# manixq/stereo_matchin

Hardware: AMD Instinct MI355X
Metric: disparity maps/sec + ms/frame, 1920×1080 d=256 ASW win=35, 1/2/4/8 MI355X (higher is better)
Workload: dtype f32

## Files before the change

include/asw.h:

```cpp
#ifndef ASW_H
#define ASW_H

#include <stddef.h>
#include <stdint.h>

#ifdef __cplusplus
extern "C" {
#endif

#define ASW_OK 0
#define ASW_E_INVALID -1
#define ASW_E_HIP -2
#define ASW_E_NOMEM -3
#define ASW_E_UNSUPPORTED -4
#define ASW_E_COMM -5

#define ASW_DIR_V 0
#define ASW_DIR_H 1

#define ASW_COLOR_RGB 0
#define ASW_COLOR_LAB 1

#define ASW_LR_U8 0
#define ASW_LR_NATIVE 1
// ... 153 lines not shown
void asw_refine_params_default(asw_refine_params *rp);
int asw_refine_params_check(const asw_params *p, const asw_refine_params *rp);
size_t asw_refine_lut_bytes(const asw_refine_params *rp);
int asw_refine_lut(const asw_params *p, const asw_refine_params *rp, float *lut, void *stream);

int asw_ref_v(const asw_params *p, const asw_refine_params *rp, const uint8_t *img_rgba, const uint8_t *est,
              int est_stride, const float *conf, const float *lut, float *out, void *stream);
int asw_ref_h(const asw_params *p, const asw_refine_params *rp, const uint8_t *img_rgba, const float *conf,
              const float *in, const float *lut, float *out, void *stream);
int asw_wta_ref(const asw_params *p, const float *cost, const float *ref_l, const float *ref_r, int32_t *d_ref,
                int32_t *d_tar, float *conf_ref, uint8_t *code_ref, uint8_t *code_tar, void *stream);
int asw_median3(const asw_params *p, const uint8_t *codes, int stride, uint8_t *out_rgba, void *stream);

size_t asw_refine_workspace_bytes(const asw_params *p, const asw_refine_params *rp);
int asw_refine(const asw_params *p, const asw_refine_params *rp, const uint8_t *left_rgba, const uint8_t *right_rgba,
               const float *cost, uint8_t *est_left_rgba, uint8_t *code_tar, float *conf_ref, float *conf_tar,
               void *workspace, uint8_t *post_red_rgba, uint8_t *final_rgba, int32_t *d_ref, int32_t *d_tar,
               void *stream);

int asw_refine_native_params_check(const asw_params *p, const asw_refine_params *rp);
int asw_refine_native_lut(const asw_params *p, const asw_refine_params *rp, float *lut, void *stream);
int asw_ref_v_native(const asw_params *p, const asw_refine_params *rp, const uint8_t *img_rgba, const int32_t *est,
                     const float *conf, const float *lut, float *out, void *stream);
int asw_consistency_native(const asw_params *p, const int32_t *d_ref, const int32_t *d_tar, float *conf_ref,
                           float *conf_tar, int32_t *est_left, uint16_t *post16, void *stream);
int asw_median3_u16(const asw_params *p, const int32_t *in, uint16_t *out, void *stream);
size_t asw_refine_native_workspace_bytes(const asw_params *p, const asw_refine_params *rp);
int asw_refine_native(const asw_params *p, const asw_refine_params *rp, const uint8_t *left_rgba,
                      const uint8_t *right_rgba, const float *cost, int32_t *est_left, int32_t *d_tar, float *conf_ref,
                      float *conf_tar, void *workspace, uint16_t *post16, uint16_t *final16, int32_t *d_ref,
                      void *stream);

typedef struct asw_cross_params {
    int arm_max;
    int tau;
} asw_cross_params;
void asw_cross_params_default(asw_cross_params *cp);
int asw_cross_params_check(const asw_params *p, const asw_cross_params *cp);
size_t asw_cross_arm_bytes(const asw_params *p);
int asw_median3_rgba(const asw_params *p, const uint8_t *in_rgba, uint8_t *out_rgba, void *stream);
int asw_cross_arms(const asw_params *p, const asw_cross_params *cp, const uint8_t *med_rgba, int8_t *arms,
                   void *stream);
int asw_cross_cost(const asw_params *p, const uint8_t *med_left_rgba, const uint8_t *med_right_rgba, float *cost,
                   void *stream);
int asw_cross_integral(const asw_params *p, int dir, float *vol, void *stream);
int asw_cross_oii(const asw_params *p, int dir, const int8_t *arms_left, const int8_t *arms_right, const float *in,
                  float *out, void *stream);
int asw_cross_init(const asw_params *p, const float *vol, int32_t *d0, uint8_t *code0, void *stream);
int asw_cross_vote(const asw_params *p, const uint8_t *code0, const int8_t *arms_left, int32_t *d1, uint8_t *code1,
                   void *stream);

#define ASW_TUNE_PASS_VARIANT 1
#define ASW_TUNE_WTA_VARIANT 2
int asw_tune_set(int key, int value);
int asw_pass_kernel(int dir, int den_mode, char *buf, int len);


typedef struct asw_ctx asw_ctx;

typedef struct asw_outputs {
    int32_t *d_ref, *d_tar;
    float *conf_ref, *conf_tar;
    uint8_t *disp_rgba;
    uint8_t *lr_rgba;
    uint8_t *lr_red_rgba;
    float *cost;
    uint8_t *final_rgba;
    uint8_t *post_red_rgba;
    uint16_t *disp16;
    uint16_t *lr16;
} asw_outputs;
#define ASW_DISP16_INVALID 0xFFFF

typedef struct asw_timings {
    double raw_cost, support, v_pass_mean, h_pass_mean, aggregation_total, wta, consistency, total;
    double h2d, d2h;
    double refine;
    double exchange;
} asw_timings;

int asw_device_name(int hip_device, char *buf, int len);

int asw_create(const asw_params *p, int hip_device, asw_ctx **out);
int asw_create_multi(const asw_params *p, const int *hip_device_ids, int n_devices, asw_ctx **out);
#define ASW_COMM_ID_BYTES 128
int asw_comm_unique_id(uint8_t id[ASW_COMM_ID_BYTES]);
int asw_create_rank(const asw_params *p, int hip_device, int rank, int nranks, const uint8_t id[ASW_COMM_ID_BYTES],
                    asw_ctx **out);
int asw_ctx_shard(const asw_ctx *ctx, int i, int *n_shards, int *d_begin, int *d_end);
int asw_destroy(asw_ctx *ctx);
int asw_match(asw_ctx *ctx, const uint8_t *left_rgba, const uint8_t *right_rgba, asw_outputs *out,
              asw_timings *t);
int asw_match_batch(asw_ctx *ctx, const uint8_t *left_rgba, const uint8_t *right_rgba, int batch,
                    asw_outputs *out, asw_timings *t);
int asw_set_refine(asw_ctx *ctx, const asw_refine_params *rp);
typedef struct asw_refine_native_outputs {
    uint16_t *final16;
    uint16_t *post16;
    int32_t *d_ref, *d_tar;
} asw_refine_native_outputs;
int asw_set_refine_native(asw_ctx *ctx, const asw_refine_params *rp, const asw_refine_native_outputs *o);
int asw_set_graph(asw_ctx *ctx, int on);
typedef struct asw_subpixel_outputs {
    float *disp;
    float *disp_lr;
    float *disp_filled;
// ... 31 lines not shown
```

stereo_matchin_amd/csrc/asw_aggregate.hip:

```cpp
#include <hip/hip_runtime.h>

#include <cstdio>
#include <cstring>
#include <mutex>

#include "asw_common.h"

namespace asw {
namespace agg {
int g_pass_variant = 0;
template <int T, int DM>
int launch_pass_tm(const asw_params *p, int dir, const float *wl, const float *wr, const float *cin, float *cout,
                   float *den, hipStream_t st, const RawSrc *raw);
template <int T, int DM>
int launch_pass32_tm(const asw_params *p, int dir, const float *wl, const float *wr, const float *cin, float *cout,
                     float *den, hipStream_t st);
template <int T, int DM>
int launch_pass32_c16_tm(const asw_params *p, const float *wl, const float *wr, const uint16_t *cin16, float *cout,
                         float *den, hipStream_t st);
template <int T>
int launch_pass32_t(const asw_params *p, int dir, const float *wl, const float *wr, const float *cin, float *cout,
                    float *den, int dm, hipStream_t st) {
    if (dm == 1) return launch_pass32_tm<T, 1>(p, dir, wl, wr, cin, cout, den, st);
    if (dm == 2) return launch_pass32_tm<T, 2>(p, dir, wl, wr, cin, cout, den, st);
    return launch_pass32_tm<T, 0>(p, dir, wl, wr, cin, cout, den, st);
}
template <int T>
int launch_pass_t(const asw_params *p, int dir, const float *wl, const float *wr, const float *cin, float *cout,
                  float *den, int dm, hipStream_t st, const RawSrc *raw) {
    if (asw_disp_pitch(p) == 32) {
        if (raw && dir == ASW_DIR_V) {
            if (dm == 1) return launch_pass32_c16_tm<T, 1>(p, wl, wr, raw->cost16, cout, den, st);
            if (dm == 0) return launch_pass32_c16_tm<T, 0>(p, wl, wr, raw->cost16, cout, den, st);
            return ASW_E_INVALID;
        }
        return launch_pass32_t<T>(p, dir, wl, wr, cin, cout, den, dm, st);
    }
    if (dm == 1) return launch_pass_tm<T, 1>(p, dir, wl, wr, cin, cout, den, st, raw);
    if (dm == 2) return launch_pass_tm<T, 2>(p, dir, wl, wr, cin, cout, den, st, raw);
    return launch_pass_tm<T, 0>(p, dir, wl, wr, cin, cout, den, st, raw);
}
}

int launch_pass_any(const asw_params *p, int dir, const float *wl, const float *wr, const float *cin, float *cout,
                    float *den, int dm, hipStream_t st);

int set_pass_variant(int v) {
    const int old = agg::g_pass_variant;
    agg::g_pass_variant = v;
    return old;
}

namespace {
std::mutex g_note_mu;
char g_note[2][3][96];
}

void note_pass_kernel(int dir, int dm, const char *kernel, int T, const char *shape, bool nt) {
    if (dir < 0 || dir > 1 || dm < 0 || dm > 2) return;
    std::lock_guard<std::mutex> lk(g_note_mu);
    std::snprintf(g_note[dir][dm], sizeof g_note[dir][dm], "%s<T=%d,%s,DM=%d%s>", kernel, T, shape, dm,
                  nt ? ",nt" : "");
}

int pass_shape_check(const asw_params *p) {
    const long long rowbytes = (long long)p->width * asw_disp_pitch(p) * 4;
    if (rowbytes * (2LL * p->taps + 16) >= (1LL << 31)) return ASW_E_UNSUPPORTED;
    if ((long long)asw_support_bytes(p) >= (1LL << 31)) return ASW_E_UNSUPPORTED;
    return ASW_OK;
}

bool ring_taps(int T) {
#ifdef ASW_DEV_TAPS
    return T == ASW_DEV_TAPS;
#else
    return T == 3 || T == 5 || T == 7 || T == 9 || T == 15 || T == 33 || T == 35 || T == 51;
#endif
}

int launch_pass(const asw_params *p, int dir, const float *wl, const float *wr, const float *cin, float *cout,
                float *den, int dm, hipStream_t st, const RawSrc *raw) {
    if (dm != 0 && !den) return ASW_E_INVALID;
    if (const int s = pass_shape_check(p)) return s;
    if (raw && (dir != ASW_DIR_V || dm == 2 || !ring_taps(p->taps))) return ASW_E_UNSUPPORTED;
#ifdef ASW_DEV_TAPS
    if (p->taps == ASW_DEV_TAPS) return agg::launch_pass_t<ASW_DEV_TAPS>(p, dir, wl, wr, cin, cout, den, dm, st, raw);
    if (raw) return ASW_E_UNSUPPORTED;
    return launch_pass_any(p, dir, wl, wr, cin, cout, den, dm, st);
#endif
    switch (p->taps) {
#define ASW_CASE(TT) \
    case TT:         \
        return agg::launch_pass_t<TT>(p, dir, wl, wr, cin, cout, den, dm, st, raw);
        ASW_CASE(3)
        ASW_CASE(5)
        ASW_CASE(7)
        ASW_CASE(9)
        ASW_CASE(15)
        ASW_CASE(33)
        ASW_CASE(35)
        ASW_CASE(51)
#undef ASW_CASE
// ... 29 lines not shown
```

stereo_matchin_amd/csrc/asw_aggregate_impl.h:

```cpp
#pragma once
#include <hip/hip_runtime.h>

#include <cstdint>
#include <type_traits>

#include "asw_common.h"

namespace asw {
namespace agg {

using f4 = float __attribute__((ext_vector_type(4)));

__device__ __forceinline__ int clampi(int v, int lo, int hi) { return v < lo ? lo : (v > hi ? hi : v); }

constexpr int kPS = 4;
constexpr int kPW = 4;

template <int B, int E, class F>
__device__ __forceinline__ void static_for(F &&f) {
    if constexpr (B < E) {
        f(std::integral_constant<int, B>{});
        static_for<B + 1, E>(f);
    }
}

__device__ __forceinline__ float div_pos(float num, float den) {
    float r = __builtin_amdgcn_rcpf(den);
    const float e = __builtin_fmaf(-den, r, 1.0f);
    r = __builtin_fmaf(e, r, r);
    float q = num * r;
    float rem = __builtin_fmaf(-den, q, num);
    q = __builtin_fmaf(rem, r, q);
    rem = __builtin_fmaf(-den, q, num);
    return __builtin_fmaf(rem, r, q);
}

template <int T>
struct Halves {
    static constexpr int QT = (T + 3) / 4;
    static constexpr int QA = (QT + 1) / 2;
    static constexpr int TA = 4 * QA < T ? 4 * QA : T;
    static constexpr int TB = T - TA;
    static constexpr int QB = QT - QA;
    static constexpr int NA = TA, NB = TB > 0 ? TB : 1;
    static constexpr int MA = QA, MB = QB > 0 ? QB : 1;
};

template <int T, int NPH>
struct Phases {
    static constexpr int QT = (T + 3) / 4;
    static constexpr int gb(int k) { return (QT * k + NPH - 1) / NPH; }
    static constexpr int tb(int k) { return 4 * gb(k) < T ? 4 * gb(k) : T; }
    static constexpr int NG = (QT + NPH - 1) / NPH;
    static constexpr int NT = 4 * NG;
};

template <int N>
__device__ __forceinline__ void wait_lgkm() {
    static_assert(N >= 0 && N < 16, "lgkmcnt field");
// ... 145 lines not shown
        const float *wlx = wlrow + xb * TP + s * TP;
        const f4 *wrx = my_slab + (xb - xs) * Q + s * Q;
        wait_lgkm0();
        asm volatile("" ::"v"(win[(s + T - 1) % U]));
        __builtin_amdgcn_sched_barrier(0);
        if constexpr (HV::TB > 0) {
            load_wl<HV::TA, T>(wlb, wlx);
            read_wr<T, HV::QA, HV::QT>(wrb, wrx);
        }
        __builtin_amdgcn_sched_barrier(0);
        float num = 1e-5f, dn = 1e-5f;
        taps<U, s, 0, HV::TA, DM != DM_READ>(num, dn, wla, wra, win);
        __builtin_amdgcn_sched_barrier(0);
        wait_lgkm0();
        __builtin_amdgcn_sched_barrier(0);
        {
            const float *pn;
            if constexpr (CHK || s == U - 1) pn = wlrow + min(x + 1, W - 1) * TP;
            else pn = wlx + TP;
            load_wl<0, HV::TA>(wla, pn);
            read_wr<T, 0, HV::QA>(wra, wrx + Q);
        }
        __builtin_amdgcn_sched_barrier(0);
        if constexpr (HV::TB > 0) taps<U, s, HV::TA, T, DM != DM_READ>(num, dn, wlb, wrb, win);
        const int xo = x * xstride;
        if constexpr (DM == DM_READ) {
            dn = dring[s % 2];
            dring[s % 2] = bload<CP>(rd, voff, min(x + 2, W - 1) * xstride);
        } else if constexpr (DM == DM_WRITE) {
            bstore<CP>(dn, rd, voff, xo);
        }
        bstore<CP>(div_pos(num, dn), ro, voff, xo);
        win[(s + U - 1) % U] = bload<CP>(rc, voff, min(x + R + P, W - 1) * xstride);
        sink += warm[s % PW];
        warm[s % PW] = wlrow[min(x + 1 + PW, W - 1) * TP + warm_off];
    };
    int xb = xw0;
    for (; xb + U <= xw1; xb += U)
        static_for<0, U>([&](auto sc) __attribute__((always_inline)) { body(sc, std::false_type{}, xb); });
    if (xb < xw1)
        static_for<0, U>([&](auto sc) __attribute__((always_inline)) { body(sc, std::true_type{}, xb); });
    if (sink == -1.0f) cout[rowoff] = sink;
}


constexpr int h11_batch(int T, int NKW) {
    return pf9_period(T) % 8 == 0 && 8 * (tap_pitch(T) / 4) <= 64 * NKW ? 8 : 4;
}
constexpr int h11_ring(int T, int NKW) { return (64 * NKW + 2 * h11_batch(T, NKW) + 15) / 16 * 16; }

template <int T, int NKW, int DM, int CP, int CPS = CP, int PX = 0, int KDH = 4>
__global__ __launch_bounds__(64 * NKW) __attribute__((amdgpu_waves_per_eu(T > 35 ? 3 : 4))) void k_hpass11(
    const float *__restrict__ wl, const float *__restrict__ wr, const float *__restrict__ cin,
    float *__restrict__ cout, float *__restrict__ den, int W, int H, int Dp, int d_begin, int nseg, int seg_len,
    int groups_per_xcd, int ngroups, int ring_off, int kbg0, int nkbg) {
    constexpr int R = T / 2;
    constexpr int TP = tap_pitch(T);
    constexpr int Q = TP / 4;
    constexpr int U = pf9_period(T) + PX;
    constexpr int P = U - T;
    constexpr int PW = 4;
    constexpr int KD = KDH;
    static_assert(U % KD == 0, "den ring period");
    constexpr int NT = 64 * NKW;
    constexpr int K = h11_batch(T, NKW);
    constexpr int RING = h11_ring(T, NKW);
    constexpr int EB = Q * 16;
    constexpr int RB = RING * EB;
    static_assert(U % K == 0 && RING >= NT + 2 * K && RING % 16 == 0, "ring geometry");
    static_assert(K * Q <= NT, "one staged float4 per thread per batch");
    __shared__ f4 ring[RING * Q];

    const int xcd = blockIdx.x & 7, m = blockIdx.x >> 3;
    const int gl = m / nkbg;
    const int g = xcd * groups_per_xcd + gl;
    if (gl >= groups_per_xcd || g >= ngroups) return;
    const int kbg = kbg0 + m - gl * nkbg;
    const int y = g / nseg;
    const int xs = (g - y * nseg) * seg_len;
    const int xe = min(xs + seg_len, W);
    const int lane = threadIdx.x & 63;
    const int wave = __builtin_amdgcn_readfirstlane(threadIdx.x >> 6);
    const int d0 = d_begin + kbg * NT;
    const int kb = kbg * NT + wave * 64;
    const float *wrrow = wr + (long long)y * W * TP;

    {
        const int e0 = xs - d0 - (NT - 1);
        for (int t = threadIdx.x; t < (NT + K) * Q; t += NT) {
            const int e = t / Q, q = t - e * Q;
            const int xr = e0 + e;
            ring[((xr + ring_off) % RING) * Q + q] =
                *reinterpret_cast<const f4 *>(wrrow + clampi(xr, 0, W - 1) * TP + 4 * q);
        }
    }
    const int st_t = min((int)threadIdx.x, K * Q - 1);
    const int st_e = st_t / Q, st_q = st_t - st_e * Q;
    int st_xr = xs + K + 1 - d0 + st_e;
    int st_addr = ((st_xr + ring_off) % RING) * EB + st_q * 16;
    f4 stg = *reinterpret_cast<const f4 *>(wrrow + clampi(st_xr, 0, W - 1) * TP + 4 * st_q);
    __syncthreads();

    const long long rowoff = (long long)y * W * Dp + kb;
    const rsrc_t rc = make_rsrc(cin + rowoff);
    const rsrc_t ro = make_rsrc(cout + rowoff);
    const rsrc_t rd = make_rsrc(den + rowoff);
    const int voff = lane * 4;
    const int xstride = Dp * 4;
    const float *wlrow = wl + (long long)y * W * TP;
    const int warm_off = lane < TP ? lane : 0;
    int ra = ((xs - d0 - wave * 64 - lane + ring_off) % RING) * EB;
    auto ring_next = [](int a) __attribute__((always_inline)) {
        const unsigned t = (unsigned)a + EB, u = t - (unsigned)RB;
        return (int)(t < u ? t : u);
    };
    auto at = [&](int a) __attribute__((always_inline)) {
        return reinterpret_cast<const f4 *>(reinterpret_cast<const char *>(ring) + a);
    };

    using HV = Halves<T>;
    float win[U];
    float wla[HV::NA], wlb[HV::NB];
    f4 wra[HV::MA], wrb[HV::MB];
    float warm[PW];
    float dring[KD];
    float sink = 0.0f;
#pragma unroll
    for (int j = 0; j < U - 1; ++j) win[j] = bload<CP>(rc, voff, clampi(xs - R + j, 0, W - 1) * xstride);
    if constexpr (DM == DM_READ) {
#pragma unroll
        for (int j = 0; j < KD; ++j) dring[j] = bload<CP>(rd, voff, min(xs + j, W - 1) * xstride);
    }
#pragma unroll
    for (int j = 0; j < PW; ++j) warm[j] = wlrow[min(xs + 1 + j, W - 1) * TP + warm_off];
    load_wl<0, HV::TA>(wla, wlrow + xs * TP);
    read_wr<T, 0, HV::QA>(wra, at(ra));

    auto body = [&](auto sc, auto chk, int xb) __attribute__((always_inline)) {
        constexpr int s = decltype(sc)::value;
        constexpr bool CHK = decltype(chk)::value;
        const int x = xb + s;
        if constexpr (CHK) {
            if (x >= xe) return;
        }
        const float *wlx = wlrow + xb * TP + s * TP;
        if constexpr (s % K == 0) {
            __syncthreads();
            *reinterpret_cast<f4 *>(reinterpret_cast<char *>(ring) + st_addr) = stg;
            st_xr += K;
            st_addr += K * EB;
            st_addr = st_addr >= RB ? st_addr - RB : st_addr;
            stg = *reinterpret_cast<const f4 *>(wrrow + clampi(st_xr, 0, W - 1) * TP + 4 * st_q);
        } else {
            wait_lgkm0();
        }
        asm volatile("" ::"v"(win[(s + T - 1) % U]));
        __builtin_amdgcn_sched_barrier(0);
        if constexpr (HV::TB > 0) {
            load_wl<HV::TA, T>(wlb, wlx);
            read_wr<T, HV::QA, HV::QT>(wrb, at(ra));
        }
        __builtin_amdgcn_sched_barrier(0);
        float num = 1e-5f, dn = 1e-5f;
        taps<U, s, 0, HV::TA, DM != DM_READ>(num, dn, wla, wra, win);
        __builtin_amdgcn_sched_barrier(0);
        wait_lgkm0();
        __builtin_amdgcn_sched_barrier(0);
        ra = ring_next(ra);
        {
            const float *pn;
            if constexpr (CHK || s == U - 1) pn = wlrow + min(x + 1, W - 1) * TP;
            else pn = wlx + TP;
            load_wl<0, HV::TA>(wla, pn);
            read_wr<T, 0, HV::QA>(wra, at(ra));
        }
        __builtin_amdgcn_sched_barrier(0);
        if constexpr (HV::TB > 0) taps<U, s, HV::TA, T, DM != DM_READ>(num, dn, wlb, wrb, win);
        const int xo = x * xstride;
        if constexpr (DM == DM_READ) {
            dn = dring[s % KD];
            dring[s % KD] = bload<CP>(rd, voff, min(x + KD, W - 1) * xstride);
        } else if constexpr (DM == DM_WRITE) {
            bstore<CPS>(dn, rd, voff, xo);
        }
        bstore<CPS>(div_pos(num, dn), ro, voff, xo);
        win[(s + U - 1) % U] = bload<CP>(rc, voff, min(x + R + P, W - 1) * xstride);
        sink += warm[s % PW];
        warm[s % PW] = wlrow[min(x + 1 + PW, W - 1) * TP + warm_off];
    };
    int xb = xs;
    for (; xb + U <= xe; xb += U)
        static_for<0, U>([&](auto sc) __attribute__((always_inline)) { body(sc, std::false_type{}, xb); });
    if (xb < xe)
        static_for<0, U>([&](auto sc) __attribute__((always_inline)) { body(sc, std::true_type{}, xb); });
    if (sink == -1.0f) cout[rowoff] = sink;
}



constexpr int ring_div(int U, int lo) {
    int n = lo;
    while (U % n != 0) ++n;
    return n;
}
constexpr int cmax(int a, int b) { return a > b ? a : b; }

template <int T, int NW, int DM, int RB, int CP, int CPS = CP, int KDV = 2, int PSV = 4, int TK = 0, int NPH = 2,
          int PX = 0, int WPE = 0, bool C16 = false>
__global__ __launch_bounds__(NW * 64) __attribute__((amdgpu_waves_per_eu(WPE ? WPE : NW >= 16 ? 4 : NW >= 12 ? 3 : 2))) void k_vpass10(
    const float *__restrict__ wl, const float *__restrict__ wr, const float *__restrict__ cin, float *__restrict__ cout,
    float *__restrict__ den, int W, int H, int Dp, int d_begin, int rows_per_strip, int nxb, int nstrip,
    int xg_per_xcd) {
    constexpr int R = T / 2;
    constexpr int TP = tap_pitch(T);
    constexpr int Q = TP / 4;
    constexpr int U = pf9_period(T) + PX;
    constexpr int P = U - T;
    constexpr int PS = PSV;
    constexpr int PW = 4;
    constexpr int KD = KDV;
    constexpr int LEAD = RB + 1;
    constexpr int NBUF = ring_div(U, 2 * RB + 1);
    static_assert(U % PS == 0 && U % PW == 0 && U % KD == 0 && U % RB == 0 && U % NBUF == 0, "ring periods");
    static_assert(LEAD <= PS, "staging ring too short for the barrier period");
    constexpr int LA = cmax(cmax(R + P, LEAD + PS), cmax(PW, KD));
    constexpr int SLAB = NW + 63;
    constexpr int NQ = SLAB * Q;
    constexpr int NSTAGE = (NQ + NW * 64 - 1) / (NW * 64);
    static_assert(NSTAGE <= 2, "slab row larger than two float4 per thread");
    __shared__ f4 slab[NBUF][NQ];

    const int nkb = Dp / 64;
    const int xcd = blockIdx.x & 7, m = blockIdx.x >> 3;
    int xg, kbi, strip;
    if constexpr (TK > 0) {
        constexpr int TCG = 32 / TK;
        const int j = m % 32, t = m / 32;
        const int ntk = (nkb + TK - 1) / TK, ntc = (xg_per_xcd + TCG - 1) / TCG;
        const int tk = t % ntk, rest = t / ntk;
        const int cgl = (rest % ntc) * TCG + j % TCG;
        kbi = tk * TK + j / TCG;
        strip = rest / ntc;
        if (cgl >= xg_per_xcd || kbi >= nkb) return;
        xg = xcd * xg_per_xcd + cgl;
    } else {
        xg = xcd * xg_per_xcd + m % xg_per_xcd;
        const int rest = m / xg_per_xcd;
// ... 155 lines not shown
                if constexpr (k == 0 && s % RB == 0) __syncthreads();
                else wait_lgkm0();
                if constexpr (k == 0) asm volatile("" ::"v"(win[(s + T - 1) % U]));
                __builtin_amdgcn_sched_barrier(0);
                if constexpr (k + 1 < NPH) {
                    request(std::integral_constant<int, k + 1>{}, wo, bcur);
                } else {
                    if constexpr (CLAMP) {
                        wo = min(y + 1, H - 1) * wrow;
                    } else {
                        wo += wrow;
                        asm volatile("" : "+s"(wo));
                    }
                    request(std::integral_constant<int, 0>{}, wo, bnext);
                }
                if constexpr (k == 0) {
                    put(bput, sa[(s + LEAD) % PS], sb[(s + LEAD) % PS]);
                    stage(sa[(s + LEAD) % PS], sb[(s + LEAD) % PS],
                          CLAMP ? min(y + LEAD + PS, H - 1) * wrow_b : soff);
                }
                __builtin_amdgcn_sched_barrier(0);
                taps<U, s, PH::tb(k), PH::tb(k + 1), DM != DM_READ>(num, dn, wlp[k], wrp[k], win);
                __builtin_amdgcn_sched_barrier(0);
            });
            if constexpr (DM == DM_READ) {
                dn = dring[s % KD];
                dring[s % KD] = bload<CP>(rdn, voff,
                                          CLAMP ? (min(y + KD, H - 1) - min(ys + KD, H - 1)) * rowbytes : so);
            } else if constexpr (DM == DM_WRITE) {
                bstore<CPS>(dn, rd, voff, so);
            }
            bstore<CPS>(div_pos(num, dn), ro, voff, so);
            if constexpr (C16) r16[s % PR] = cload_raw(rc, CLAMP ? (min(y + R + P, H - 1) - cb) * rowbytes : so);
            else win[(s + U - 1) % U] = cload(rc, CLAMP ? (min(y + R + P, H - 1) - cb) * rowbytes : so);
            sink += warm[s % PW];
            warm[s % PW] = bload(rwl, warm_voff, CLAMP ? min(y + PW, H - 1) * wrow_b : woff);
            so += rowbytes;
            woff += wrow_b;
            soff += wrow_b;
            asm volatile("" : "+s"(so), "+s"(woff), "+s"(soff));
        });
    };
    int ys = y_begin;
    for (; ys + U <= y_end && ys + U - 1 + LA <= H - 1; ys += U) chunk(std::integral_constant<int, 0>{}, ys);
    for (; ys + U <= y_end; ys += U) {
        asm volatile("" : "+s"(ys));
        chunk(std::integral_constant<int, 1>{}, ys);
    }
    if (ys < y_end) chunk(std::integral_constant<int, 2>{}, ys);
    if (sink == -1.0f) cout[kb + lane] = sink;
}

extern int g_pass_variant;

template <int T, int NW, int DM, int RB = 2, int CP = 0, int CPS = CP, int PS = 4, int NPH = 2, bool C16 = false,
          int TK = 0>
void launch_v10(const asw_params *p, const float *wl, const float *wr, const float *cin, float *cout, float *den,
                hipStream_t st, const RawSrc *raw = nullptr) {
    constexpr int U = pf9_period(T);
    const int W = p->width, H = p->height;
    const int Dp = asw_disp_pitch(p);
    const int nkb = Dp / 64;
    const int nxb = (W + NW - 1) / NW;
    int nstrip = (int)((2048LL + (long long)nxb * nkb - 1) / ((long long)nxb * nkb));
    const int max_strip = H / (2 * T) > 1 ? H / (2 * T) : 1;
    if (nstrip > max_strip) nstrip = max_strip;
    if (nstrip < 1) nstrip = 1;
    const int rows = ((H + nstrip - 1) / nstrip + U - 1) / U * U;
    nstrip = (H + rows - 1) / rows;
    const int per_xcd = (nxb + 7) / 8;
    constexpr int TCG = TK > 0 ? 32 / TK : 1;
    const int nblocks = TK > 0 ? 8 * 32 * ((nkb + TK - 1) / (TK > 0 ? TK : 1)) * ((per_xcd + TCG - 1) / TCG) * nstrip
                               : 8 * per_xcd * nkb * nstrip;
    hipLaunchKernelGGL((k_vpass10<T, NW, DM, RB, CP, CPS, 2, PS, TK, NPH, 0, 0, C16>), dim3(nblocks), dim3(NW * 64), 0,
                       st, wl, wr, C16 ? reinterpret_cast<const float *>(raw->cost16) : cin, cout, den, W, H, Dp,
                       p->d_begin, rows, nxb, nstrip, per_xcd);
    const char *shape = NW == 16 ? (NPH == 2 ? "NW=16" : "NW=16,NPH>2")
                        : NW == 12 ? (NPH == 2 ? "NW=12" : TK == 4 ? "NW=12,NPH=3,TK=4" : "NW=12,NPH=3") : "NW=8";
    note_pass_kernel(ASW_DIR_V, DM, C16 ? "k_vpass10_c16" : "k_vpass10", T, shape, CP == kCPStream);
}

template <int T, int NW, int XW, int DM, int CP = 0>
void launch_h9(const asw_params *p, const float *wl, const float *wr, const float *cin, float *cout, float *den,
               hipStream_t st) {
    const int W = p->width, H = p->height;
    const int Dp = asw_disp_pitch(p);
    const int nkb = Dp / 64;
    constexpr int SEG = NW * XW;
    const int nseg = (W + SEG - 1) / SEG;
    const int nblocks = (H * nseg + 7) / 8 * 8 * nkb;
    hipLaunchKernelGGL((k_hpass9<T, NW, XW, DM, CP>), dim3(nblocks), dim3(NW * 64), 0, st, wl, wr, cin, cout, den, W, H,
                       Dp, p->d_begin, nseg);
    note_pass_kernel(ASW_DIR_H, DM, "k_hpass9", T, "NW=4", CP == kCPStream);
}

template <int T, int NKW, int DM, int CP, int CPS = CP, int PX = 0, int KDH = 4>
void launch_h11(const asw_params *p, const float *wl, const float *wr, const float *cin, float *cout, float *den,
                hipStream_t st, int seg_len) {
#ifndef ASW_PASS_EXP_FORMS
    static_assert(NKW == 4 || NKW == 2 || NKW == 1, "no label for this block shape");
    static_assert(PX == 0 || (NKW == 2 && PX == 24), "the PX=24 label names the 2-block form with PX = 24");
#endif
    constexpr int RING = h11_ring(T, NKW);
    const int W = p->width, H = p->height;
    const int Dp = asw_disp_pitch(p);
    const int nkbg = Dp / (64 * NKW);
    const int nseg = (W + seg_len - 1) / seg_len;
    const int ngroups = H * nseg;
    const int per_xcd = (ngroups + 7) / 8;
    const int ring_off = ((p->d_begin + Dp) / RING + 1) * RING;
    hipLaunchKernelGGL((k_hpass11<T, NKW, DM, CP, CPS, PX, KDH>), dim3(8 * per_xcd * nkbg), dim3(64 * NKW), 0, st, wl, wr, cin,
                       cout, den, W, H, Dp, p->d_begin, nseg, seg_len, per_xcd, ngroups, ring_off, 0, nkbg);
    note_pass_kernel(ASW_DIR_H, DM, "k_hpass11", T,
                     NKW == 4 ? "NKW=4" : NKW == 2 ? (PX ? "NKW=2,PX=24" : "NKW=2") : "NKW=1", CP == kCPStream);
}

inline bool v12_tiles(const asw_params *p) {
    const int nxb = (p->width + 11) / 12;
    return asw_disp_pitch(p) / 64 >= 4 && (nxb + 7) / 8 >= 8;
}

template <int T, int DM>
void launch_dm(const asw_params *p, int dir, const float *wl, const float *wr, const float *cin, float *cout,
               float *den, hipStream_t st, const RawSrc *raw) {
    constexpr int U9 = pf9_period(T);
    constexpr int XW9 = U9 * (64 / U9 > 1 ? 64 / U9 : 1);
    const int v = g_pass_variant;
    bool stream = (long long)p->width * p->height * asw_disp_pitch(p) * 4 >= (256LL << 20);
    if (v & (1 << 26)) stream = !stream;
    if (raw) {
        if constexpr (DM != DM_READ) {
            if constexpr (T <= 35) {
                if (stream) launch_v10<T, 16, DM, 2, kCPStream, kCPStream, 4, 2, true>(p, wl, wr, cin, cout, den, st, raw);
                else launch_v10<T, 16, DM, 2, 0, 0, 4, 2, true>(p, wl, wr, cin, cout, den, st, raw);
            } else {
                if (stream && v12_tiles(p)) launch_v10<T, 12, DM, 2, kCPStream, kCPStream, 4, 3, true, 4>(p, wl, wr, cin, cout, den, st, raw);
                else if (stream) launch_v10<T, 12, DM, 2, kCPStream, kCPStream, 4, 3, true>(p, wl, wr, cin, cout, den, st, raw);
                else launch_v10<T, 12, DM, 2, 0, 0, 4, 3, true>(p, wl, wr, cin, cout, den, st, raw);
            }
        }
        return;
    }
    if (dir == ASW_DIR_V) {
        if (stream) {
            if constexpr (T <= 35) launch_v10<T, 16, DM, 2, kCPStream>(p, wl, wr, cin, cout, den, st);
            else if (v12_tiles(p)) launch_v10<T, 12, DM, 2, kCPStream, kCPStream, 4, 3, false, 4>(p, wl, wr, cin, cout, den, st);
            else launch_v10<T, 12, DM, 2, kCPStream, kCPStream, 4, 3>(p, wl, wr, cin, cout, den, st);
        } else {
            if constexpr (T <= 35) launch_v10<T, 16, DM, 2, 0>(p, wl, wr, cin, cout, den, st);
            else launch_v10<T, 12, DM, 2, 0, 0, 4, 3>(p, wl, wr, cin, cout, den, st);
        }
    } else {
        const int nkb = asw_disp_pitch(p) / 64;
        const int seg = h11_seg_len(T, v);
        if (h11_selected(p, v)) {
            if constexpr (T <= 35) {
                if (nkb % 4 == 0) launch_h11<T, 4, DM, kCPStream>(p, wl, wr, cin, cout, den, st, seg);
                else if (nkb % 2 == 0) launch_h11<T, 2, DM, kCPStream>(p, wl, wr, cin, cout, den, st, seg);
                else launch_h11<T, 1, DM, kCPStream>(p, wl, wr, cin, cout, den, st, seg);
            } else if constexpr (T == 51 && DM == DM_READ) {
                constexpr int PXH = 24;
                const int seg51 = (v >> 8) & 15 ? seg : 4 * (pf9_period(T) + PXH);
                if (nkb % 2 == 0) launch_h11<T, 2, DM, kCPStream, kCPStream, PXH>(p, wl, wr, cin, cout, den, st, seg51);
                else launch_h11<T, 1, DM, kCPStream>(p, wl, wr, cin, cout, den, st, seg);
            } else {
                if (nkb % 2 == 0) launch_h11<T, 2, DM, kCPStream>(p, wl, wr, cin, cout, den, st, seg);
                else launch_h11<T, 1, DM, kCPStream>(p, wl, wr, cin, cout, den, st, seg);
            }
        } else if (stream) {
            launch_h9<T, 4, XW9, DM, kCPStream>(p, wl, wr, cin, cout, den, st);
        } else {
            launch_h9<T, 4, XW9, DM>(p, wl, wr, cin, cout, den, st);
        }
    }
}

template <int T, int DM>
int launch_pass_tm(const asw_params *p, int dir, const float *wl, const float *wr, const float *cin, float *cout,
                   float *den, hipStream_t st, const RawSrc *raw) {
    launch_dm<T, DM>(p, dir, wl, wr, cin, cout, den, st, raw);
    const hipError_t e = hipGetLastError();
    if (e != hipSuccess) {
        set_hip_error(e);
        return ASW_E_HIP;
    }
    return ASW_OK;
}

}
}

#define ASW_INSTANTIATE_PASS(TT, DM)                                                                                 \
    template int asw::agg::launch_pass_tm<TT, DM>(const asw_params *, int, const float *, const float *,            \
                                                  const float *, float *, float *, hipStream_t, const RawSrc *);
```

stereo_matchin_amd/csrc/asw_common.h:

```cpp
#pragma once
#include <hip/hip_runtime.h>

#include "asw.h"

namespace asw {

constexpr int kWave = 64;
constexpr int kSadMax = 765;
constexpr int kLutWidth = kSadMax + 1;

__host__ __device__ constexpr int tap_pitch(int T) {
    int k = (T + 3) / 4;
    if ((k & 1) == 0) ++k;
    return 4 * k;
}

__host__ __device__ constexpr int round_up(int v, int m) { return (v + m - 1) / m * m; }

__host__ __device__ inline int code_u8(int d, int D) {
    if (D <= 1) return 0;
    long long c = (510LL * d + (D - 2)) / (2LL * (D - 1));
    return c > 255 ? 255 : (c < 0 ? 0 : (int)c);
}

__device__ __forceinline__ bool lr_consistent(int mode, int D, long long p, int dr, const int32_t *d_tar,
                                              const uint8_t *code_ref, const uint8_t *code_tar) {
    if (mode == ASW_LR_U8) {
        const float scale = (float)(D - 1);
        const float qr = ((float)code_ref[p] / 255.0f) * scale;
        const float qt = ((float)code_tar[p] / 255.0f) * scale;
        return fabsf(qt - qr) < 1.001f;
    }
    const int dd = dr - d_tar[p];
    return dd <= 1 && dd >= -1;
}

void set_hip_error(hipError_t e);

__host__ __device__ inline int d_end_of_p(const asw_params *p) { return p->d_end < 0 ? p->ndisp : p->d_end; }

struct RawSrc {
    const uint16_t *cost16;
};

int launch_pass(const asw_params *p, int dir, const float *wl, const float *wr, const float *cin, float *cout,
                float *den, int dm, hipStream_t st, const RawSrc *raw = nullptr);
int h11_seg_len(int T, int variant);
bool h11_selected(const asw_params *p, int variant);
bool ring_taps(int T);
int set_pass_variant(int v);
constexpr int kPassVariantBits = 128 | 4096 | 0xF00;
void note_pass_kernel(int dir, int dm, const char *kernel, int T, const char *shape, bool nt);
int pass_shape_check(const asw_params *p);

int raw_cost16_check(const asw_params *p);
int census_cost16_check(const asw_params *p, const asw_census_params *cp);
int sgm_shape_check(const asw_params *p);

int launch_wta_local_scan(const asw_params *p, const float *cost, const float *ref, long long *key, float *m1,
                          float *m2, hipStream_t st);
int launch_wta_target_local_scan(const asw_params *p, const float *cost, const long long *key_ref, const float *ref,
                                 long long *tkey, float *t1, float *t2, hipStream_t st);
int launch_wta_scan(const asw_params *p, int mode, const float *cost, const float *ref_l, const float *ref_r,
                    int32_t *d_ref, float *conf_ref, int32_t *d_tar, float *conf_tar, uint8_t *code_ref,
                    uint8_t *code_tar, hipStream_t st);

}
```

stereo_matchin_amd/csrc/asw_kernels.hip:

```cpp
#include <hip/hip_runtime.h>

#include <climits>
#include <cstdint>

#include "asw_common.h"
#include "asw_srgb_table.h"

namespace asw {

static thread_local int g_last_hip_error = 0;
void set_hip_error(hipError_t e) { g_last_hip_error = (int)e; }

namespace {

__device__ __forceinline__ int clampi(int v, int lo, int hi) { return v < lo ? lo : (v > hi ? hi : v); }

__device__ double exp_d(double x) {
    const double inv_ln2 = 1.44269504088896338700e+00;
    const double ln2_hi = 6.93147180369123816490e-01;
    const double ln2_lo = 1.90821492927058770002e-10;
    const double k = rint(x * inv_ln2);
    double r = fma(-k, ln2_hi, x);
    r = fma(-k, ln2_lo, r);
    double p = 1.0 / 87178291200.0;
// ... 316 lines not shown
                              uchar4 *__restrict__ out_red) {
    const long long p = (long long)blockIdx.x * blockDim.x + threadIdx.x;
    if (p >= n) return;
    const uint8_t cr = code_ref[p], ct = code_tar[p];
    bool cons;
    if (mode == ASW_LR_U8) {
        const float scale = (float)(D - 1);
        const float qr = ((float)cr / 255.0f) * scale;
        const float qt = ((float)ct / 255.0f) * scale;
        cons = fabsf(qt - qr) < 1.001f;
    } else {
        const int dd = d_ref[p] - d_tar[p];
        cons = dd <= 1 && dd >= -1;
    }
    if (!cons) {
        conf_ref[p] = 0.0f;
        conf_tar[p] = 0.0f;
    }
    if (out) out[p] = cons ? make_uchar4(cr, cr, cr, 255) : make_uchar4(ct, ct, ct, 255);
    if (out_red) out_red[p] = cons ? make_uchar4(cr, cr, cr, 255) : make_uchar4(255, 0, 0, 255);
}

inline int finish_launch() {
    const hipError_t e = hipGetLastError();
    if (e != hipSuccess) {
        set_hip_error(e);
        return ASW_E_HIP;
    }
    return ASW_OK;
}


}
}

using namespace asw;

namespace asw {
int launch_wta_sweep(const asw_params *p, const float *cost, int32_t *d_ref, float *conf_ref, int32_t *d_tar,
                     float *conf_tar, uint8_t *code_ref, uint8_t *code_tar, hipStream_t st);
}

extern "C" {

int asw_abi_version(void) { return ASW_ABI_VERSION; }

static int g_wta_variant = 0;

int asw_tune_set(int key, int value) {
    if (key == ASW_TUNE_PASS_VARIANT) {
        if (value & ~(asw::kPassVariantBits | 0xFF0000 | (1 << 26))) return ASW_E_INVALID;
        return asw::set_pass_variant(value);
    }
    if (key == ASW_TUNE_WTA_VARIANT) {
        if (value != 0 && value != 2) return ASW_E_INVALID;
        const int old = g_wta_variant;
        g_wta_variant = value;
        return old;
    }
    return ASW_E_INVALID;
}

void asw_params_default(asw_params *p) {
    if (!p) return;
    p->width = 0;
    p->height = 0;
    p->ndisp = 61;
    p->taps = 33;
    p->iters = 7;
    p->gamma_c = 30.91f;
    p->gamma_g = 28.21f;
    p->color_space = ASW_COLOR_RGB;
    p->tad_tau = 765.0f;
    p->lr_check = 1;
    p->lr_mode = ASW_LR_U8;
    p->d_begin = 0;
    p->d_end = -1;
    p->flags = 0;
}

static inline int d_end_of(const asw_params *p) { return p->d_end < 0 ? p->ndisp : p->d_end; }

int asw_params_check(const asw_params *p) {
    if (!p) return ASW_E_INVALID;
    if (p->width < 1 || p->height < 1 || p->ndisp < 1 || p->taps < 1 || (p->taps & 1) == 0) return ASW_E_INVALID;
    if (p->iters < 0 || !(p->gamma_c > 0.0f) || !(p->gamma_g > 0.0f)) return ASW_E_INVALID;
    if (p->d_begin < 0 || d_end_of(p) > p->ndisp || p->d_begin >= d_end_of(p)) return ASW_E_INVALID;
    if (p->color_space != ASW_COLOR_RGB && p->color_space != ASW_COLOR_LAB) return ASW_E_INVALID;
    if (p->lr_mode != ASW_LR_U8 && p->lr_mode != ASW_LR_NATIVE) return ASW_E_INVALID;
    if ((long long)p->width * p->height > (1LL << 31) / 64) return ASW_E_INVALID;
    if (p->flags & ~ASW_FLAG_ALL) return ASW_E_INVALID;
    return ASW_OK;
}

const char *asw_strerror(int s) {
    switch (s) {
        case ASW_OK: return "ok";
        case ASW_E_INVALID: return "invalid parameter";
        case ASW_E_HIP: return "HIP runtime error";
        case ASW_E_NOMEM: return "out of memory";
        case ASW_E_UNSUPPORTED: return "unsupported parameter combination";
        case ASW_E_COMM: return "collective (RCCL) error";
        default: return "unknown status";
    }
}

// ... 297 lines not shown
```

Before: 44.54.

## Split horizontal pass into persistent balanced row-range work per occupancy slot

Changes the h11 horizontal aggregation kernel from one block per fixed row segment into persistent blocks that each walk a balanced contiguous range of column units across rows. The range count defaults to the occupancy-derived number of resident slots, queried once per device and cached. This aims to cut block launch overhead, avoid the tail of partially filled waves, and let rows be processed with full-length segments that amortise the ring warm-up. In exchange, each row change re-warms the ring and register windows inside the loop, adds extra syncs, and the load balance depends on the occupancy query.

```diff
diff --git a/include/asw.h b/include/asw.h
--- a/include/asw.h
+++ b/include/asw.h
@@ -229,6 +229,7 @@
 
 #define ASW_TUNE_PASS_VARIANT 1
 #define ASW_TUNE_WTA_VARIANT 2
+#define ASW_TUNE_H_RANGES 3
 int asw_tune_set(int key, int value);
 int asw_pass_kernel(int dir, int den_mode, char *buf, int len);
 
diff --git a/stereo_matchin_amd/csrc/asw_aggregate.hip b/stereo_matchin_amd/csrc/asw_aggregate.hip
--- a/stereo_matchin_amd/csrc/asw_aggregate.hip
+++ b/stereo_matchin_amd/csrc/asw_aggregate.hip
@@ -9,6 +9,7 @@
 namespace asw {
 namespace agg {
 int g_pass_variant = 0;
+int g_h_ranges = 0;
 template <int T, int DM>
 int launch_pass_tm(const asw_params *p, int dir, const float *wl, const float *wr, const float *cin, float *cout,
                    float *den, hipStream_t st, const RawSrc *raw);
@@ -48,6 +49,12 @@
 int set_pass_variant(int v) {
     const int old = agg::g_pass_variant;
     agg::g_pass_variant = v;
+    return old;
+}
+
+int set_h_ranges(int n) {
+    const int old = agg::g_h_ranges;
+    agg::g_h_ranges = n;
     return old;
 }
 
diff --git a/stereo_matchin_amd/csrc/asw_aggregate_impl.h b/stereo_matchin_amd/csrc/asw_aggregate_impl.h
--- a/stereo_matchin_amd/csrc/asw_aggregate_impl.h
+++ b/stereo_matchin_amd/csrc/asw_aggregate_impl.h
@@ -1,10 +1,12 @@
 #pragma once
 #include <hip/hip_runtime.h>
 
+#include <atomic>
 #include <cstdint>
 #include <type_traits>
 
 #include "asw_common.h"
+#include "asw_h11_split.h"
 
 namespace asw {
 namespace agg {
@@ -256,8 +258,8 @@
 template <int T, int NKW, int DM, int CP, int CPS = CP, int PX = 0, int KDH = 4>
 __global__ __launch_bounds__(64 * NKW) __attribute__((amdgpu_waves_per_eu(T > 35 ? 3 : 4))) void k_hpass11(
     const float *__restrict__ wl, const float *__restrict__ wr, const float *__restrict__ cin,
-    float *__restrict__ cout, float *__restrict__ den, int W, int H, int Dp, int d_begin, int nseg, int seg_len,
-    int groups_per_xcd, int ngroups, int ring_off, int kbg0, int nkbg) {
+    float *__restrict__ cout, float *__restrict__ den, int W, int H, int Dp, int d_begin, int cpr, int cw,
+    int ranges_per_xcd, int nranges, int ring_off, int kbg0, int nkbg) {
     constexpr int R = T / 2;
     constexpr int TP = tap_pitch(T);
     constexpr int Q = TP / 4;
@@ -276,44 +278,18 @@
     __shared__ f4 ring[RING * Q];
 
     const int xcd = blockIdx.x & 7, m = blockIdx.x >> 3;
-    const int gl = m / nkbg;
-    const int g = xcd * groups_per_xcd + gl;
-    if (gl >= groups_per_xcd || g >= ngroups) return;
-    const int kbg = kbg0 + m - gl * nkbg;
-    const int y = g / nseg;
-    const int xs = (g - y * nseg) * seg_len;
-    const int xe = min(xs + seg_len, W);
-    const int lane = threadIdx.x & 63;
+    const int rl = m / nkbg;
+    const int r = xcd * ranges_per_xcd + rl;
+    if (rl >= ranges_per_xcd || r >= nranges) return;
+    const int kbg = kbg0 + m - rl * nkbg;
+    const long long C = (long long)H * cpr;
+    const int c1 = (int)h11_range_begin(r + 1, nranges, C);
+    int c = (int)h11_range_begin(r, nranges, C);
     const int wave = __builtin_amdgcn_readfirstlane(threadIdx.x >> 6);
     const int d0 = d_begin + kbg * NT;
     const int kb = kbg * NT + wave * 64;
-    const float *wrrow = wr + (long long)y * W * TP;
-
-    {
-        const int e0 = xs - d0 - (NT - 1);
-        for (int t = threadIdx.x; t < (NT + K) * Q; t += NT) {
-            const int e = t / Q, q = t - e * Q;
-            const int xr = e0 + e;
-            ring[((xr + ring_off) % RING) * Q + q] =
-                *reinterpret_cast<const f4 *>(wrrow + clampi(xr, 0, W - 1) * TP + 4 * q);
-        }
-    }
-    const int st_t = min((int)threadIdx.x, K * Q - 1);
-    const int st_e = st_t / Q, st_q = st_t - st_e * Q;
-    int st_xr = xs + K + 1 - d0 + st_e;
-    int st_addr = ((st_xr + ring_off) % RING) * EB + st_q * 16;
-    f4 stg = *reinterpret_cast<const f4 *>(wrrow + clampi(st_xr, 0, W - 1) * TP + 4 * st_q);
-    __syncthreads();
-
-    const long long rowoff = (long long)y * W * Dp + kb;
-    const rsrc_t rc = make_rsrc(cin + rowoff);
-    const rsrc_t ro = make_rsrc(cout + rowoff);
-    const rsrc_t rd = make_rsrc(den + rowoff);
-    const int voff = lane * 4;
+    const int voff = (threadIdx.x & 63) * 4;
     const int xstride = Dp * 4;
-    const float *wlrow = wl + (long long)y * W * TP;
-    const int warm_off = lane < TP ? lane : 0;
-    int ra = ((xs - d0 - wave * 64 - lane + ring_off) % RING) * EB;
     auto ring_next = [](int a) __attribute__((always_inline)) {
         const unsigned t = (unsigned)a + EB, u = t - (unsigned)RB;
         return (int)(t < u ? t : u);
@@ -321,82 +297,118 @@
     auto at = [&](int a) __attribute__((always_inline)) {
         return reinterpret_cast<const f4 *>(reinterpret_cast<const char *>(ring) + a);
     };
-
     using HV = Halves<T>;
-    float win[U];
-    float wla[HV::NA], wlb[HV::NB];
-    f4 wra[HV::MA], wrb[HV::MB];
-    float warm[PW];
-    float dring[KD];
     float sink = 0.0f;
-#pragma unroll
-    for (int j = 0; j < U - 1; ++j) win[j] = bload<CP>(rc, voff, clampi(xs - R + j, 0, W - 1) * xstride);
-    if constexpr (DM == DM_READ) {
-#pragma unroll
-        for (int j = 0; j < KD; ++j) dring[j] = bload<CP>(rd, voff, min(xs + j, W - 1) * xstride);
-    }
-#pragma unroll
-    for (int j = 0; j < PW; ++j) warm[j] = wlrow[min(xs + 1 + j, W - 1) * TP + warm_off];
-    load_wl<0, HV::TA>(wla, wlrow + xs * TP);
-    read_wr<T, 0, HV::QA>(wra, at(ra));
-
-    auto body = [&](auto sc, auto chk, int xb) __attribute__((always_inline)) {
-        constexpr int s = decltype(sc)::value;
-        constexpr bool CHK = decltype(chk)::value;
-        const int x = xb + s;
-        if constexpr (CHK) {
-            if (x >= xe) return;
-        }
-        const float *wlx = wlrow + xb * TP + s * TP;
-        if constexpr (s % K == 0) {
-            __syncthreads();
-            *reinterpret_cast<f4 *>(reinterpret_cast<char *>(ring) + st_addr) = stg;
-            st_xr += K;
-            st_addr += K * EB;
-            st_addr = st_addr >= RB ? st_addr - RB : st_addr;
-            stg = *reinterpret_cast<const f4 *>(wrrow + clampi(st_xr, 0, W - 1) * TP + 4 * st_q);
-        } else {
+    long long rowoff = kb;
+
+    while (c < c1) {
+        const H11Piece pc = h11_piece(c, c1, cpr, cw, W);
+        c += pc.n;
+        const int y = pc.y, xs = pc.xs, xe = pc.xe;
+        const float *wrrow = wr + (long long)y * W * TP;
+        int lane4 = voff;
+        asm volatile("" : "+v"(lane4));
+        const int lane = (int)((unsigned)lane4 >> 2), tid = wave * 64 + lane;
+        const int warm_off = lane < TP ? lane : 0;
+        const int st_t = min(tid, K * Q - 1);
+        const int st_e = st_t / Q, st_q = st_t - st_e * Q;
+
+        __syncthreads();
+        {
+            const int e0 = xs - d0 - (NT - 1);
+            for (int t = tid; t < (NT + K) * Q; t += NT) {
+                const int e = t / Q, q = t - e * Q;
+                const int xr = e0 + e;
+                ring[((xr + ring_off) % RING) * Q + q] =
+                    *reinterpret_cast<const f4 *>(wrrow + clampi(xr, 0, W - 1) * TP + 4 * q);
+            }
+        }
+        int st_xr = xs + K + 1 - d0 + st_e;
+        int st_addr = ((st_xr + ring_off) % RING) * EB + st_q * 16;
+        f4 stg = *reinterpret_cast<const f4 *>(wrrow + clampi(st_xr, 0, W - 1) * TP + 4 * st_q);
+        __syncthreads();
+
+        rowoff = (long long)y * W * Dp + kb;
+        const rsrc_t rc = make_rsrc(cin + rowoff);
+        const rsrc_t ro = make_rsrc(cout + rowoff);
+        const rsrc_t rd = make_rsrc(den + rowoff);
+        const float *wlrow = wl + (long long)y * W * TP;
+        int ra = ((xs - d0 - wave * 64 - lane + ring_off) % RING) * EB;
+
+        float win[U];
+        float wla[HV::NA], wlb[HV::NB];
+        f4 wra[HV::MA], wrb[HV::MB];
+        float warm[PW];
+        float dring[KD];
+#pragma unroll
+        for (int j = 0; j < U - 1; ++j) win[j] = bload<CP>(rc, voff, clampi(xs - R + j, 0, W - 1) * xstride);
+        if constexpr (DM == DM_READ) {
+#pragma unroll
+            for (int j = 0; j < KD; ++j) dring[j] = bload<CP>(rd, voff, min(xs + j, W - 1) * xstride);
+        }
+#pragma unroll
+        for (int j = 0; j < PW; ++j) warm[j] = wlrow[min(xs + 1 + j, W - 1) * TP + warm_off];
+        load_wl<0, HV::TA>(wla, wlrow + xs * TP);
+        read_wr<T, 0, HV::QA>(wra, at(ra));
+
+        auto body = [&](auto sc, auto chk, int xb) __attribute__((always_inline)) {
+            constexpr int s = decltype(sc)::value;
+            constexpr bool CHK = decltype(chk)::value;
+            const int x = xb + s;
+            if constexpr (CHK) {
+                if (x >= xe) return;
+            }
+            const float *wlx = wlrow + xb * TP + s * TP;
+            if constexpr (s % K == 0) {
+                __syncthreads();
+                *reinterpret_cast<f4 *>(reinterpret_cast<char *>(ring) + st_addr) = stg;
+                st_xr += K;
+                st_addr += K * EB;
+                st_addr = st_addr >= RB ? st_addr - RB : st_addr;
+                stg = *reinterpret_cast<const f4 *>(wrrow + clampi(st_xr, 0, W - 1) * TP + 4 * st_q);
+            } else {
+                wait_lgkm0();
+            }
+            asm volatile("" ::"v"(win[(s + T - 1) % U]));
+            __builtin_amdgcn_sched_barrier(0);
+            if constexpr (HV::TB > 0) {
+                load_wl<HV::TA, T>(wlb, wlx);
+                read_wr<T, HV::QA, HV::QT>(wrb, at(ra));
+            }
+            __builtin_amdgcn_sched_barrier(0);
+            float num = 1e-5f, dn = 1e-5f;
+            taps<U, s, 0, HV::TA, DM != DM_READ>(num, dn, wla, wra, win);
+            __builtin_amdgcn_sched_barrier(0);
             wait_lgkm0();
-        }
-        asm volatile("" ::"v"(win[(s + T - 1) % U]));
-        __builtin_amdgcn_sched_barrier(0);
-        if constexpr (HV::TB > 0) {
-            load_wl<HV::TA, T>(wlb, wlx);
-            read_wr<T, HV::QA, HV::QT>(wrb, at(ra));
-        }
-        __builtin_amdgcn_sched_barrier(0);
-        float num = 1e-5f, dn = 1e-5f;
-        taps<U, s, 0, HV::TA, DM != DM_READ>(num, dn, wla, wra, win);
-        __builtin_amdgcn_sched_barrier(0);
-        wait_lgkm0();
-        __builtin_amdgcn_sched_barrier(0);
-        ra = ring_next(ra);
-        {
-            const float *pn;
-            if constexpr (CHK || s == U - 1) pn = wlrow + min(x + 1, W - 1) * TP;
-            else pn = wlx + TP;
-            load_wl<0, HV::TA>(wla, pn);
-            read_wr<T, 0, HV::QA>(wra, at(ra));
-        }
-        __builtin_amdgcn_sched_barrier(0);
-        if constexpr (HV::TB > 0) taps<U, s, HV::TA, T, DM != DM_READ>(num, dn, wlb, wrb, win);
-        const int xo = x * xstride;
-        if constexpr (DM == DM_READ) {
-            dn = dring[s % KD];
-            dring[s % KD] = bload<CP>(rd, voff, min(x + KD, W - 1) * xstride);
-        } else if constexpr (DM == DM_WRITE) {
-            bstore<CPS>(dn, rd, voff, xo);
-        }
-        bstore<CPS>(div_pos(num, dn), ro, voff, xo);
-        win[(s + U - 1) % U] = bload<CP>(rc, voff, min(x + R + P, W - 1) * xstride);
-        sink += warm[s % PW];
-        warm[s % PW] = wlrow[min(x + 1 + PW, W - 1) * TP + warm_off];
-    };
-    int xb = xs;
-    for (; xb + U <= xe; xb += U)
-        static_for<0, U>([&](auto sc) __attribute__((always_inline)) { body(sc, std::false_type{}, xb); });
-    if (xb < xe)
-        static_for<0, U>([&](auto sc) __attribute__((always_inline)) { body(sc, std::true_type{}, xb); });
+            __builtin_amdgcn_sched_barrier(0);
+            ra = ring_next(ra);
+            {
+                const float *pn;
+                if constexpr (CHK || s == U - 1) pn = wlrow + min(x + 1, W - 1) * TP;
+                else pn = wlx + TP;
+                load_wl<0, HV::TA>(wla, pn);
+                read_wr<T, 0, HV::QA>(wra, at(ra));
+            }
+            __builtin_amdgcn_sched_barrier(0);
+            if constexpr (HV::TB > 0) taps<U, s, HV::TA, T, DM != DM_READ>(num, dn, wlb, wrb, win);
+            const int xo = x * xstride;
+            if constexpr (DM == DM_READ) {
+                dn = dring[s % KD];
+                dring[s % KD] = bload<CP>(rd, voff, min(x + KD, W - 1) * xstride);
+            } else if constexpr (DM == DM_WRITE) {
+                bstore<CPS>(dn, rd, voff, xo);
+            }
+            bstore<CPS>(div_pos(num, dn), ro, voff, xo);
+            win[(s + U - 1) % U] = bload<CP>(rc, voff, min(x + R + P, W - 1) * xstride);
+            sink += warm[s % PW];
+            warm[s % PW] = wlrow[min(x + 1 + PW, W - 1) * TP + warm_off];
+        };
+        int xb = xs;
+        for (; xb + U <= xe; xb += U)
+            static_for<0, U>([&](auto sc) __attribute__((always_inline)) { body(sc, std::false_type{}, xb); });
+        if (xb < xe)
+            static_for<0, U>([&](auto sc) __attribute__((always_inline)) { body(sc, std::true_type{}, xb); });
+    }
     if (sink == -1.0f) cout[rowoff] = sink;
 }
 
@@ -658,6 +670,7 @@
 }
 
 extern int g_pass_variant;
+extern int g_h_ranges;
 
 template <int T, int NW, int DM, int RB = 2, int CP = 0, int CPS = CP, int PS = 4, int NPH = 2, bool C16 = false,
           int TK = 0>
@@ -708,15 +721,37 @@
     static_assert(PX == 0 || (NKW == 2 && PX == 24), "the PX=24 label names the 2-block form with PX = 24");
 #endif
     constexpr int RING = h11_ring(T, NKW);
+    constexpr int U = pf9_period(T) + PX;
+    const auto kernel = k_hpass11<T, NKW, DM, CP, CPS, PX, KDH>;
     const int W = p->width, H = p->height;
     const int Dp = asw_disp_pitch(p);
     const int nkbg = Dp / (64 * NKW);
-    const int nseg = (W + seg_len - 1) / seg_len;
-    const int ngroups = H * nseg;
-    const int per_xcd = (ngroups + 7) / 8;
+    const int cw = seg_len > 0 ? seg_len : U;
+    const int cpr = h11_units_per_row(W, cw);
+    const long long C = (long long)H * cpr;
+    long long nranges = C;
+    if (seg_len <= 0) {
+        nranges = g_h_ranges;
+        if (nranges <= 0) {
+            constexpr int kDevs = 64;
+            static std::atomic<int> slots_of[kDevs];
+            int dev = 0, slots = 0;
+            if (hipGetDevice(&dev) != hipSuccess) return;
+            if (dev >= 0 && dev < kDevs) slots = slots_of[dev].load(std::memory_order_relaxed);
+            if (slots == 0) {
+                int per_cu = 0, cus = 0;
+                if (hipOccupancyMaxActiveBlocksPerMultiprocessor(&per_cu, kernel, 64 * NKW, 0) != hipSuccess) return;
+                if (hipDeviceGetAttribute(&cus, hipDeviceAttributeMultiprocessorCount, dev) != hipSuccess) return;
+                slots = per_cu * cus > 0 ? per_cu * cus : 1;
+                if (dev >= 0 && dev < kDevs) slots_of[dev].store(slots, std::memory_order_relaxed);
+            }
+            nranges = slots / nkbg > 0 ? slots / nkbg : 1;
+        }
+    }
+    const int per_xcd = (int)((nranges + 7) / 8);
     const int ring_off = ((p->d_begin + Dp) / RING + 1) * RING;
-    hipLaunchKernelGGL((k_hpass11<T, NKW, DM, CP, CPS, PX, KDH>), dim3(8 * per_xcd * nkbg), dim3(64 * NKW), 0, st, wl, wr, cin,
-                       cout, den, W, H, Dp, p->d_begin, nseg, seg_len, per_xcd, ngroups, ring_off, 0, nkbg);
+    hipLaunchKernelGGL(kernel, dim3(8 * per_xcd * nkbg), dim3(64 * NKW), 0, st, wl, wr, cin, cout, den, W, H, Dp,
+                       p->d_begin, cpr, cw, per_xcd, (int)nranges, ring_off, 0, nkbg);
     note_pass_kernel(ASW_DIR_H, DM, "k_hpass11", T,
                      NKW == 4 ? "NKW=4" : NKW == 2 ? (PX ? "NKW=2,PX=24" : "NKW=2") : "NKW=1", CP == kCPStream);
 }
@@ -758,7 +793,7 @@
         }
     } else {
         const int nkb = asw_disp_pitch(p) / 64;
-        const int seg = h11_seg_len(T, v);
+        const int seg = (v >> 8) & 15 ? h11_seg_len(T, v) : 0;
         if (h11_selected(p, v)) {
             if constexpr (T <= 35) {
                 if (nkb % 4 == 0) launch_h11<T, 4, DM, kCPStream>(p, wl, wr, cin, cout, den, st, seg);
@@ -766,8 +801,7 @@
                 else launch_h11<T, 1, DM, kCPStream>(p, wl, wr, cin, cout, den, st, seg);
             } else if constexpr (T == 51 && DM == DM_READ) {
                 constexpr int PXH = 24;
-                const int seg51 = (v >> 8) & 15 ? seg : 4 * (pf9_period(T) + PXH);
-                if (nkb % 2 == 0) launch_h11<T, 2, DM, kCPStream, kCPStream, PXH>(p, wl, wr, cin, cout, den, st, seg51);
+                if (nkb % 2 == 0) launch_h11<T, 2, DM, kCPStream, kCPStream, PXH>(p, wl, wr, cin, cout, den, st, seg);
                 else launch_h11<T, 1, DM, kCPStream>(p, wl, wr, cin, cout, den, st, seg);
             } else {
                 if (nkb % 2 == 0) launch_h11<T, 2, DM, kCPStream>(p, wl, wr, cin, cout, den, st, seg);
diff --git a/stereo_matchin_amd/csrc/asw_common.h b/stereo_matchin_amd/csrc/asw_common.h
--- a/stereo_matchin_amd/csrc/asw_common.h
+++ b/stereo_matchin_amd/csrc/asw_common.h
@@ -49,6 +49,7 @@
 bool h11_selected(const asw_params *p, int variant);
 bool ring_taps(int T);
 int set_pass_variant(int v);
+int set_h_ranges(int n);
 constexpr int kPassVariantBits = 128 | 4096 | 0xF00;
 void note_pass_kernel(int dir, int dm, const char *kernel, int T, const char *shape, bool nt);
 int pass_shape_check(const asw_params *p);
diff --git a/stereo_matchin_amd/csrc/asw_h11_split.h b/stereo_matchin_amd/csrc/asw_h11_split.h
--- /dev/null
+++ b/stereo_matchin_amd/csrc/asw_h11_split.h
@@ -0,0 +1,30 @@
+#pragma once
+
+#if defined(__HIPCC__) || defined(__CUDACC__)
+#define ASW_H11_HD __host__ __device__
+#else
+#define ASW_H11_HD
+#endif
+
+namespace asw {
+
+ASW_H11_HD inline int h11_units_per_row(int W, int cw) { return (W + cw - 1) / cw; }
+
+ASW_H11_HD inline long long h11_range_begin(long long r, long long N, long long C) { return r * C / N; }
+
+struct H11Piece {
+    int y, xs, xe;
+    int n;
+};
+
+ASW_H11_HD inline H11Piece h11_piece(int c, int c1, int cpr, int cw, int W) {
+    H11Piece pc;
+    pc.y = c / cpr;
+    const int cc = c - pc.y * cpr;
+    pc.n = c1 - c < cpr - cc ? c1 - c : cpr - cc;
+    pc.xs = cc * cw;
+    pc.xe = pc.xs + pc.n * cw < W ? pc.xs + pc.n * cw : W;
+    return pc;
+}
+
+}
diff --git a/stereo_matchin_amd/csrc/asw_kernels.hip b/stereo_matchin_amd/csrc/asw_kernels.hip
--- a/stereo_matchin_amd/csrc/asw_kernels.hip
+++ b/stereo_matchin_amd/csrc/asw_kernels.hip
@@ -392,6 +392,10 @@
         if (value & ~(asw::kPassVariantBits | 0xFF0000 | (1 << 26))) return ASW_E_INVALID;
         return asw::set_pass_variant(value);
     }
+    if (key == ASW_TUNE_H_RANGES) {
+        if (value < 0) return ASW_E_INVALID;
+        return asw::set_h_ranges(value);
+    }
     if (key == ASW_TUNE_WTA_VARIANT) {
         if (value != 0 && value != 2) return ASW_E_INVALID;
         const int old = g_wta_variant;
```

Result: slower. 43.66 (-2.0%).
